# josephg/text-crdt-rust

Measured on AMD Instinct MI355X. Metric: CRDT ops remapped+merged/sec (whole node), higher is better.
Workload: dtype u32

## Files before the change

### text-crdt-rust_amd/csrc/host_plan.h

```cpp
#pragma once
#include <algorithm>
#include <cstring>
#include <string>
#include <unordered_map>
#include <vector>

#include "crdt_types.h"

namespace crdt {

struct WireTxnView {
  u32 agent_name, seq, n_parents, n_ops;
  const u32* parents;
  const u32* ops;
};
struct WireView {
  std::vector<std::string> names;
  std::vector<WireTxnView> txns;
  bool parse(const uint8_t* p, size_t len) {
    size_t off = 0;
    auto rd = [&](u32& v) -> bool {
      if (off + 4 > len) return false;
      std::memcpy(&v, p + off, 4);
      off += 4;
      return true;
    };
    u32 magic, nn;
    if (!rd(magic) || magic != 0x31585452u || !rd(nn)) return false;
    names.resize(nn);
    for (u32 i = 0; i < nn; i++) {
      u32 bl;
      if (!rd(bl) || off + bl > len) return false;
      names[i].assign((const char*)p + off, bl);
      off += (bl + 3) & ~3u;
    }
    u32 nt;
    if (!rd(nt)) return false;
    if (off % 4) return false;
    txns.resize(nt);
    for (u32 t = 0; t < nt; t++) {
      WireTxnView& x = txns[t];
      if (!rd(x.agent_name) || !rd(x.seq) || !rd(x.n_parents) || !rd(x.n_ops)) return false;
      if (x.agent_name >= nn) return false;
      if (off + 8ull * x.n_parents + 24ull * x.n_ops > len) return false;
      x.parents = (const u32*)(p + off);
      off += 8ull * x.n_parents;
      x.ops = (const u32*)(p + off);
      off += 24ull * x.n_ops;
      for (u32 k = 0; k < x.n_parents; k++) if (x.parents[2 * k] >= nn) return false;
      for (u32 k = 0; k < x.n_ops; k++) {
        const u32* o = x.ops + 6 * k;
        if (o[0] > 1 || o[1] >= nn || (o[0] == 0 && o[3] >= nn)) return false;
      }
    }
    return true;
  }
};

struct AgentTable {
  std::vector<std::string> names;
  std::unordered_map<std::string, u32> ids;
  u32 get_or_create(const std::string& n) {
    if (n == "ROOT") return ROOT_AGENT;
    auto it = ids.find(n);
    if (it != ids.end()) return it->second;
    u32 id = (u32)names.size();
    names.push_back(n);
    ids[n] = id;
    return id;
  }
  u32 lookup(const std::string& n) const {
    if (n == "ROOT") return ROOT_AGENT;
    auto it = ids.find(n);
    return it == ids.end() ? UNKNOWN_AGENT : it->second;
  }
  std::vector<u32> ranks() const {
    std::vector<u32> idx(names.size());
    for (u32 i = 0; i < idx.size(); i++) idx[i] = i;
    std::sort(idx.begin(), idx.end(), [&](u32 a, u32 b) { return names[a] < names[b]; });
    std::vector<u32> r(names.size());
    for (u32 i = 0; i < idx.size(); i++) r[idx[i]] = i;
    return r;
  }
};

struct StreamNeeds {
  u64 n_txn = 0, n_ltxn = 0, n_rtxn = 0, n_ops = 0, orders = 0, local_del = 0, remote_del_ops = 0, remote_parents = 0;
  u32 max_ops = 0, max_del = 0, max_len = 0, max_parents = 0;
  u64 probes = 0;
  u64 local_del_ops = 0;
  u32 max_rdel_len = 0;
  std::vector<u32> txns_per_agent;
  void txn_max(u32 ops, u64 del, u64 len, u32 parents) {
    max_ops = std::max(max_ops, ops);
    max_del = (u32)std::min<u64>(std::max<u64>(max_del, del), 0xFFFFFFFFull);
    max_len = (u32)std::min<u64>(std::max<u64>(max_len, len), 0xFFFFFFFFull);
    max_parents = std::max(max_parents, parents);
  }
  void agent_txn(u32 a) {
    if (a >= 0xFFFE) return;
    if (txns_per_agent.size() <= a) txns_per_agent.resize(a + 1, 0);
    txns_per_agent[a]++;
  }
};

inline void encode_lc(std::vector<Rec>& out, StreamNeeds& nd, u32 agent, u32 pos, u32 del, u32 ins) {
  out.push_back(Rec{(REC_LC << 28) | agent, pos, del, ins});
  nd.txn_max(1, del, (u64)del + ins, 0);
  nd.local_del += del;
  nd.local_del_ops += del != 0;
  nd.n_txn++;
  nd.n_ltxn++;
  nd.n_ops++;
  nd.orders += (u64)del + ins;
  nd.agent_txn(agent);
}
inline void encode_local_txn(std::vector<Rec>& out, StreamNeeds& nd, u32 agent, const u32* ops3, u32 nops) {
  u64 span = 0, dels = 0;
  for (u32 k = 0; k < nops; k++) { span += (u64)ops3[3 * k + 1] + ops3[3 * k + 2]; dels += ops3[3 * k + 1]; }
  u32 span32 = span > 0xFFFFFFFFull ? 0xFFFFFFFFu : (u32)span;
  u32 dels32 = dels > 0xFFFFFFFFull ? 0xFFFFFFFFu : (u32)dels;
  if (agent <= 0xFFFFu && span != 0 && span <= 0xFFFFFFFFull &&
      (nops > 1 || (ops3[1] != 0 && ops3[2] != 0))) {
    for (u32 k = 0; k < nops; k++) {
      u32 pos = ops3[3 * k], del = ops3[3 * k + 1], ins = ops3[3 * k + 2];
      if (del) encode_lc(out, nd, agent, pos, del, 0);
      if (ins) encode_lc(out, nd, agent, pos, 0, ins);
    }
    return;
  }
  nd.txn_max(nops, dels, span, 0);
  if (nops == 1 && agent <= 0xFFFFu && span <= 0xFFFFFFFFull) {
    out.push_back(Rec{(REC_LC << 28) | agent, ops3[0], ops3[1], ops3[2]});
    nd.local_del += ops3[1];
    nd.local_del_ops += ops3[1] != 0;
  } else {
    out.push_back(Rec{(REC_LTXN << 28) | (nops & 0x0FFFFFFFu), agent, dels32, span32});
    for (u32 k = 0; k < nops; k++) {
      out.push_back(Rec{REC_LOP << 28, ops3[3 * k], ops3[3 * k + 1], ops3[3 * k + 2]});
      nd.local_del += ops3[3 * k + 1];
      nd.local_del_ops += ops3[3 * k + 1] != 0;
    }
  }
  nd.n_txn++;
  nd.n_ltxn++;
  nd.n_ops += nops;
  nd.orders += span;
  nd.agent_txn(agent);
}

inline void encode_remote(std::vector<Rec>& out, StreamNeeds& nd, AgentTable& at, const WireView& wv) {
  std::vector<u32> cache(wv.names.size(), 0xFFFFFFFFu);
  for (const WireTxnView& t : wv.txns) {
    size_t before = at.names.size();
    u32 author = at.get_or_create(wv.names[t.agent_name]);
    if (at.names.size() != before)
      for (u32 i = 0; i < cache.size(); i++) if (cache[i] == UNKNOWN_AGENT) cache[i] = 0xFFFFFFFFu;
    auto res = [&](u32 ni) -> u32 {
      if (cache[ni] == 0xFFFFFFFFu) cache[ni] = at.lookup(wv.names[ni]);
      return cache[ni];
    };
    u64 tl = 0;
    bool zero = false;
    for (u32 k = 0; k < t.n_ops; k++) {
      u32 len = t.ops[6 * k + 5];
      if (len == 0 || len > 0x0FFFFFFFu) zero = true;
      tl += len;
    }
    u32 tl32 = tl > 0xFFFFFFFFull ? 0xFFFFFFFFu : (u32)tl;
    nd.txn_max(t.n_ops, t.n_ops, tl, t.n_parents);
    u32 has_del = 0;
    for (u32 k = 0; k < t.n_ops; k++)
      if (t.ops[6 * k] != 0) { has_del = 1; nd.max_rdel_len = std::max<u32>(nd.max_rdel_len, tl32); break; }
    if (t.n_ops == 1 && t.n_parents == 1 && author < 0xFFFEu && t.seq >= 1 && res(t.parents[0]) == author &&
        t.parents[1] == t.seq - 1) {
      const u32* o = t.ops;
      u32 len = o[5];
      auto org = [&](u32 ni, u32 seq, u32& enc) -> bool {
        u32 a = res(ni);
        if (a == ROOT_AGENT) { enc = 0xFFFFFFFFu; return true; }
        enc = seq;
        return a == author && seq != 0xFFFFFFFFu;
      };
      u32 e2 = 0, e3 = 0;
      bool ok = len >= 1 && len <= 0x7FFu;
      if (ok && o[0] == 0) ok = org(o[1], o[2], e2) && org(o[3], o[4], e3);
      else if (ok) ok = res(o[1]) == author && o[2] != 0xFFFFFFFFu && (e2 = o[2], true);
      if (ok) {
        out.push_back(Rec{(REC_RC << 28) | ((o[0] ? 1u : 0u) << 27) | (len << 16) | author, t.seq, e2, e3});
        if (o[0]) nd.remote_del_ops++;
        nd.n_txn++;
        nd.n_rtxn++;
        nd.n_ops += 1;
        nd.orders += tl;
        nd.remote_parents += 1;
        nd.agent_txn(author);
        continue;
      }
    }
    if (t.n_ops > RTXN_NOPS_MASK) zero = true;
    out.push_back(Rec{(REC_RTXN << 28) | ((zero ? 1u : 0u) << 27) | (has_del << RTXN_DEL_BIT) | (t.n_ops & RTXN_NOPS_MASK),
                      (author & 0xFFFFu) | ((t.n_parents & 0xFFFFu) << 16), t.seq, tl32});
    for (u32 k = 0; k < t.n_ops; k++) {
      const u32* o = t.ops + 6 * k;
      u32 len = o[5] & 0x0FFFFFFFu;
      if (o[0] == 0) {
        out.push_back(Rec{(REC_RINS << 28) | len, (res(o[1]) & 0xFFFFu) | ((res(o[3]) & 0xFFFFu) << 16), o[2], o[4]});
      } else {
        out.push_back(Rec{(REC_RDEL << 28) | len, res(o[1]) & 0xFFFFu, o[2], 0});
        nd.remote_del_ops++;
      }
    }
    for (u32 k = 0; k < t.n_parents; k++)
      out.push_back(Rec{REC_RPARENT << 28, res(t.parents[2 * k]) & 0xFFFFu, t.parents[2 * k + 1], 0});
    nd.n_txn++;
    nd.n_rtxn++;
    nd.n_ops += t.n_ops;
    nd.orders += tl;
    nd.remote_parents += t.n_parents;
    nd.agent_txn(author);
  }
}

inline void encode_probe(std::vector<Rec>& out, StreamNeeds& nd, u32 pos, u32 agent, u32 seq) {
  out.push_back(Rec{REC_PROBE << 28, pos, agent, seq});
  nd.probes++;
}

inline void encode_gen(std::vector<Rec>& out, StreamNeeds& nd, u32 agent, u32 n_ops, u32 seed) {
  out.push_back(Rec{REC_GEN << 28, agent, n_ops, seed});
  nd.txn_max(1, 10, 10, 0);
  nd.n_txn += n_ops;
  nd.n_ltxn += n_ops;
  nd.n_ops += n_ops;
  nd.orders += 3ull * n_ops;
  nd.local_del += n_ops;
  nd.local_del_ops += n_ops;
  if (agent < 0xFFFE) {
    if (nd.txns_per_agent.size() <= agent) nd.txns_per_agent.resize(agent + 1, 0);
    nd.txns_per_agent[agent] += n_ops;
  }
}

constexpr u32 MAX_LEAVES = 32u * 32u * (ROOT_CAP_MAX - 64u);

struct Caps {
  u32 leaf, blk, map, cwo, arun, del, dd, txn, par, agent, fr;
  u32 ord;
  u32 canon = 0;
};
inline u32 blk_cap_for(u32 leaf_cap) { return leaf_cap / 32 + 2; }
inline u32 root_cap_for(u32 blk_cap) {
  u32 r = (blk_cap + 63u) & ~63u;
  return r < ROOT_CAP_MIN ? ROOT_CAP_MIN : r;
}
inline Caps plan_caps(const StreamNeeds& nd, u32 n_agents, bool track, u32 leaf_div = 48) {
  Caps c;
  u64 leaves = 64 + nd.n_ops / leaf_div;
  c.leaf = (u32)std::min<u64>(leaves, 1 + 2 * nd.n_ops + 1);
  if (c.leaf < 64) c.leaf = 64;
  if (c.leaf > MAX_LEAVES) c.leaf = MAX_LEAVES;
  c.blk = blk_cap_for(c.leaf);
  c.fr = FRONTIER_CAP0;
  c.map = track ? (u32)std::min<u64>(nd.orders + 1, 0xFFFFFFFFull) : 0;
  c.ord = (u32)std::min<u64>(nd.orders + 1, 0xFFFFFFFFull);
  c.cwo = (u32)std::min<u64>(nd.n_txn + 1, 256 + nd.n_txn / 64);
  c.txn = c.cwo;
  u64 arun = 0;
  for (u32 a = 0; a < n_agents; a++) arun += (a < nd.txns_per_agent.size() ? nd.txns_per_agent[a] : 0) + 1;
  c.arun = (u32)arun;
  c.del = (u32)std::min<u64>(std::min<u64>(nd.local_del + nd.remote_del_ops, 2 * (nd.local_del_ops + nd.remote_del_ops) + 64) + 1,
                             0xFFFFFFFFull);
  c.dd = nd.remote_del_ops ? std::max<u32>(4u, (u32)std::min<u64>((2ull * nd.max_rdel_len + 2) / 32 + 3, 0x7FFFFFFFull)) : 0u;
  c.par = (u32)std::min<u64>(nd.remote_parents + nd.n_txn + 64 + 1, 1024 + (nd.remote_parents + nd.n_txn) / 64);
  c.agent = n_agents;
  return c;
}

}
```

### text-crdt-rust_amd/csrc/replay_core.h

```cpp
#pragma once
#include "crdt_types.h"

namespace crdt {

struct Cursor {
  u32 leaf, idx, off;
};
constexpr u32 END_LEAF = 0xFFFFFFFEu;

enum : u32 {
  P_LV = 0, P_DL = 2, P_DV = 4, P_SOL = 6, P_LOF = 8, P_CWO = 10, P_ARUN = 12, P_DELS = 14,
  P_DD = 16, P_TXNS = 18, P_PAR = 20, P_FR = 22, P_AGENTS = 24, P_GROUPS = 26, P_RECS = 28, P_STP = 30,
  P_DDB = 32,
  P_PROBE = P_DDB + 2,
  K_LEAF = P_PROBE + 2, K_MAP, K_CWO, K_TXN, K_DEL, K_DD, K_PAR, K_RECN,
  K_FR,
  P_OAG,
  K_AGMAP = P_OAG + 2,
  P_LAG,
  S_BASE = 64,
  S_STATUS = 64, S_REC_POS, S_N_LEAVES, S_N_BLOCKS, S_NG, S_NEXT_ORDER, S_LEN, S_N_CWO, S_N_DEL,
  S_N_DD, S_N_TXN, S_N_PAR, S_N_FR, S_N_AGENTS, S_N_ITEMS, S_CAP_NEED, S_N_ENTRIES, S_GEN_DONE, S_N_DDB,
  S_PROF0, S_PROF1, S_PROF2, S_PROF3,
  F_FAST,
// ... 1428 lines not shown
    u32 pos0 = g(T_RB_BASE) + b0;
    u32 end = g(T_RB_BASE) + nv;
    while (true) {
      if (pos0 + (nt + 1u) * per <= end) break;
      if (end >= rn) break;
      u32 last = pos0 + (nt - 1u) * per;
      u32 n = rn - last < 64u ? rn - last : 64u;
      u32 t2, l0;
      u32 n2 = w.typing_scan_at(w.at(recs(), last), n, remote, cpt, agent, ow1, o.w3, t2, l0);
      end = last + n;
      if (n2 <= 1u) break;
      total += t2 - l0;
      nt += n2 - 1u;
    }
    return nt;
  }
  CRDT_HD u32 fast_typing(u32 b0, u32 nv, u32 remote, u32 idx, u32 orr, u32 agent, const Rec& o, u32 first) {
    Span e = w.cget(idx);
    if (e.len <= 0) return 0;
    if (e.order + (u32)e.len != first) return 0;
    if (e.orr != orr) return 0;
    u32 total;
    u32 nt = typing_run(b0, nv, remote, agent, o.w1, o, total);
    if (g(K_MAP) - first < total) return 0;
    map_fill(first, total, g(C_LEAF));
    e.len += (i32)total;
    w.cset(idx, e);
    p(C_NOW, g(C_NOW) + total);
    p(C_DIRTY, 1u);
    fast_txn_commit(first, total);
    return nt * per_txn(remote);
  }
  CRDT_HD u32 leaf_delete(u32 idx, u32 off, u32 l) {
    Span e = w.cget(idx);
    u32 n = g(C_N);
    u32 target = e.order + off;
    u32 ha = off > 0u, hc = off + l < (u32)e.len;
    Span pa{e.order, e.ol, e.orr, (i32)off};
    Span dd{target, ha ? target - 1u : e.ol, e.orr, -(i32)l};
    Span pc{target + l, target + l - 1u, e.orr, e.len - (i32)(off + l)};
    Span x0 = ha ? dd : pc;
    u32 m = ha + hc;
    u32 pre = 0;
    Span nx{0, 0, 0, 0};
    if (m != 0u) {
      if (idx + 1u < n) {
        nx = w.cget(idx + 1u);
        Span last = m == 2u ? pc : x0;
        if (can_append_u(last, nx)) {
          nx.order = last.order;
          nx.len += last.len;
          pre = 1;
          m -= 1u;
        }
      }
    }
    if (n + m > (u32)L) return 0;
    w.cset(idx, ha ? pa : dd);
    if (pre) w.cset(idx + 1u, nx);
    if (m) {
      w.cache_shift_right(idx + 1u, n, m);
      p(C_N, n + m);
      w.cset(idx + 1u, x0);
      if (m == 2u) w.cset(idx + 2u, pc);
      inc(S_N_ENTRIES, m);
    }
    p(C_NOW, g(C_NOW) - l);
    p(C_DIRTY, 1u);
    return 1;
  }
  CRDT_HD u32 delete_run_closed(u32 idx, u32 off, u32 t1, u32 k, u32 back) {
    Span E = w.cget(idx);
    u32 n = g(C_N);
    u32 orr = E.orr;
    u32 has_nx = idx + 1u < n;
    Span N0 = w.cget(idx + 1u);
    u32 room = (u32)L - n;
    u32 delta;
    if (back) {
      u32 mid = off + 1u != (u32)E.len ? 1u : 0u;
      u32 p0 = 0u;
      if (mid) {
        if (room == 0u) return 0;
        room -= 1u;
      } else if (has_nx) {
        p0 = can_append_u(Span{t1, t1 - 1u, orr, -1}, N0) ? 1u : 0u;
      }
      u32 kmax = 2u * room + p0;
      k = k < off ? k : off;
      k = k < kmax ? k : kmax;
      if (k < 2u) return 0;
      if (mid) {
        Span pc = truncate(E, off + 1u);
        w.cache_shift_right(idx + 1u, n, 1u);
        w.cset(idx + 1u, pc);
        n += 1u;
        inc(S_N_ENTRIES, 1u);
      }
      delta = p0 ? k / 2u : (k + 1u) / 2u;
      w.cache_shift_right(idx + 1u, n, delta);
      w.cset_lanes(idx + 1u, idx + 1u + delta, [&](u32 lane) {
        u32 q = delta - (lane - idx - 1u);
        u32 jc = p0 ? 2u * q : 2u * q - 1u;
        u32 tc = t1 - (jc - 1u);
        u32 two = jc + 1u <= k ? 1u : 0u;
        return Span{tc - two, tc - 1u, orr, (i32)~two};
      });
      if (p0) w.cset(idx + 1u + delta, Span{t1, N0.ol, N0.orr, N0.len - 1});
      E.len = (i32)(off + 1u - k);
      w.cset(idx, E);
    } else {
      u32 ha = off > 0u;
      if (has_nx && can_append_u(Span{t1 + 1u, t1, orr, E.len - (i32)off - 1}, N0)) return 0;
      u32 kmax = room > ha ? room - ha : 0u;
      k = k < kmax ? k : kmax;
      if (k < 2u) return 0;
      u32 rest = (u32)E.len - off - k;
      u32 cnt = ha + k + (rest != 0u);
      delta = cnt - 1u;
      w.cache_shift_right(idx + 1u, n, delta);
      w.cset_lanes(idx, idx + cnt, [&](u32 lane) {
        u32 p = lane - idx;
        u32 j = p - ha;
        if (ha && p == 0u) return Span{E.order, E.ol, orr, (i32)off};
        if (j < k) return Span{t1 + j, (j == 0u && !ha) ? E.ol : t1 + j - 1u, orr, -1};
        return Span{t1 + k, t1 + k - 1u, orr, (i32)rest};
      });
    }
    p(C_N, n + delta);
    inc(S_N_ENTRIES, delta);
    p(C_NOW, g(C_NOW) - k);
    p(C_DIRTY, 1u);
    return k;
  }
  CRDT_HD u32 fast_deletes(u32 b0, u32 nv, u32 remote, u32 agent, u32 idx, u32 off, u32 l, u32 first, const Rec& o) {
#ifdef CRDT_PROF
    u64 pt0 = w.clock();
#endif
    u32 per = per_txn(remote);
    u32 t1 = w.cget_order(idx) + off;
    u32 split_first = 0;
    if (g(C_N) + 2u > (u32)L) {
      Span e = w.cget(idx);
      u32 n = g(C_N), ha = off > 0u, hc = off + l < (u32)e.len, m = ha + hc;
      if (m && idx + 1u < n) {
        Span last = hc ? Span{t1 + l, t1 + l - 1u, e.orr, e.len - (i32)(off + l)}
                       : Span{t1, ha ? t1 - 1u : e.ol, e.orr, -(i32)l};
        m -= can_append_u(last, w.cget(idx + 1u));
      }
      if (n + m > (u32)L) split_first = 1;
    }
    u32 k = 1, back = 0;
    u32 key = g(T_AGL_KEY);
    u32 delta;
    u32 has_next = b0 + 2u * per <= nv ? 1u : 0u;
    u32 bn = has_next ? b0 + per : b0;
    if (cpt) {
      Rec r2 = w.rec_get(bn);
      delta = remote ? r2.w2 - o.w2 : r2.w1 - o.w1;
    } else {
      Rec o2 = op_at(bn, remote);
      delta = remote ? o2.w2 - o.w2 : o2.w1 - o.w1;
    }
    u32 bk = delta == 0xFFFFFFFFu ? 1u : 0u;
    u32 bad = (l ^ 1u) | (has_next ^ 1u) | ((delta != (remote ? 1u : 0u) ? 1u : 0u) & (bk ^ 1u));
    if (remote) bad |= ((o.w1 & 0xFFFFu) ^ agent) | (o.w2 - key >= g(T_AGL_LEN) ? 1u : 0u);
    if (opq(bad) == 0u) {
      back = opq(bk);
      {
        u32 room = back ? off + 1u : (u32)w.cget_len(idx) - off;
        if (remote) {
          u32 r2 = back ? o.w2 - key + 1u : key + g(T_AGL_LEN) - o.w2;
          room = room < r2 ? room : r2;
        }
        k = w.delete_scan(b0, nv, remote, cpt, agent, delta);
        u32 rn = rec_n();
        u32 pos0 = g(T_RB_BASE) + b0;
        u32 end = g(T_RB_BASE) + nv;
        while (true) {
          if (k >= room) break;
          if (pos0 + (k + 1u) * per <= end) break;
          if (end >= rn) break;
          u32 last = pos0 + (k - 1u) * per;
          u32 n = rn - last < 64u ? rn - last : 64u;
          u32 n2 = w.delete_scan_at(w.at(recs(), last), n, remote, cpt, agent, delta);
          end = last + n;
          if (n2 <= 1u) break;
          k += n2 - 1u;
        }
#ifdef CRDT_PROF

#endif
        k = k < room ? k : room;
      }
    }
#ifdef CRDT_PROF

#endif
    if (g(K_MAP) - first < k * l) return 0;
    if (g(K_DEL) - g(S_N_DEL) < (back ? k : 1u)) return 0;
#ifdef CRDT_PROF
    u64 pt1 = w.clock();
#endif
    u32 done = split_first ? 0u : delete_segment(idx, off, t1, k, back, l);
#ifdef CRDT_PROF
    u64 pt2 = w.clock();
#endif
    CRDT_STAT(9, 1); CRDT_STAT(12, k); CRDT_STAT(13, split_first);
#ifdef CRDT_PROF_LOOP
    u32 lp_gen = 0, lp_split = 0, lp_find = 0, lp_seg = 0;
#endif
    while (done < k) {
#ifdef CRDT_PROF_LOOP
      u64 q0 = w.clock();
#endif
      CRDT_STAT(10, 1);
      if (g(K_LEAF) - g(S_N_LEAVES) < 2u) break;
      Cursor c{g(C_LEAF), idx, off};
      if (done != 0u) {
        if (!find_order(back ? t1 - done : t1 + done, true, c)) break;
      }
      i32 el = w.cget_len(c.idx);
      if (el <= 0) break;
      if (c.off + l > (u32)el) break;
      if (back & (el == 1)) {
        w.cset_len(c.idx, -1);
        p(C_NOW, g(C_NOW) - 1u);
        p(C_DIRTY, 1u);
        done++;
        continue;
      }
      CRDT_STAT(back ? 48 : 49, 1); CRDT_STAT(52, c.off == 0u);
#ifdef CRDT_PROF_LOOP
      u64 q1 = w.clock();
      prof_split = 0;
#endif
      delete_general(c.idx, c.off, l, back);
#ifdef CRDT_PROF_LOOP
      u64 q2 = w.clock();
      lp_gen += (u32)(q2 - q1) - prof_split;
      lp_split += prof_split;
      lp_find += (u32)(q1 - q0);
#endif
      done++;
      if (done == k) break;
      u32 t2 = back ? t1 - done : t1 + done;
      if (back & (c.off != 0u)) c.off -= 1u;
      else if (!find_order(t2, true, c)) break;
      el = w.cget_len(c.idx);
      if (el <= 0) break;
      if (c.off + l > (u32)el) break;
#ifdef CRDT_PROF_LOOP
      u64 q3 = w.clock();
      lp_find += (u32)(q3 - q2);
#endif
      if (back & (c.leaf == g(C_LEAF)) & (l == 1u)) {
        u32 dc = back_cycles(c.idx, t2, k - done);
        CRDT_STAT(57, dc != 0u); CRDT_STAT(58, dc);
        if (dc) {
          done += dc;
          if (done == k) break;
          t2 -= dc;
          c.off -= dc;
        }
      }
      u32 dseg = delete_segment(c.idx, c.off, t2, k - done, back, l);
#ifdef CRDT_PROF_LOOP
      lp_seg += (u32)(w.clock() - q3);
#endif
      CRDT_STAT(53, dseg); CRDT_STAT(54, dseg == 0u);
      done += dseg;
    }
#ifdef CRDT_PROF
    u64 pt3 = w.clock();
#endif
    if (done == 0u) return 0;
    if (back) {
      append_delete(first, t1, 1u);
      if (done > 1u) {
        u32 n = g(S_N_DEL);
        w.st(&w.at(dels(), n - 1u)->len, g(T_DEL_LEN));
        w.st_del_run(w.at(dels(), n), done - 1u, first + 1u, t1 - 1u);
        p(S_N_DEL, n + done - 1u);
        p(T_DEL_KEY, first + done - 1u);
        p(T_DEL_ORDER, t1 - (done - 1u));
        p(T_DEL_LEN, 1u);
      }
    } else {
      append_delete(first, t1, done * l);
    }
    fast_txn_commit(first, done * l);
#ifdef CRDT_PROF
    if (prof_mode == 3u && !prof_gen) {
#ifdef CRDT_PROF_LOOP
      (void)pt0; (void)pt1; (void)pt2; (void)pt3;
      inc(S_PROF0, lp_gen); inc(S_PROF1, lp_split); inc(S_PROF2, lp_find); inc(S_PROF3, lp_seg);
#else
      inc(S_PROF0, (u32)(pt1 - pt0)); inc(S_PROF1, (u32)(pt2 - pt1));
      inc(S_PROF2, (u32)(pt3 - pt2)); inc(S_PROF3, (u32)(w.clock() - pt3));
#endif
    }
#endif
    return done * per;
  }
  CRDT_HD u32 delete_segment(u32 idx, u32 off, u32 t, u32 k, u32 back, u32 l) {
    u32 done = k >= 2u ? delete_run_closed(idx, off, t, k, back) : 0u;
    CRDT_STAT(11, done); CRDT_STAT(14, 1);
    if (done == 0u) {
      for (u32 j = 0; j < k; j++) {
        u32 ij = back ? idx : (j == 0u ? idx : idx + (off > 0u) + j);
        u32 oj = back ? off - j : (j == 0u ? off : 0u);
        u32 tj = back ? t - j : t + j;
        if (w.cget_order(ij) + oj != tj) break;
        if (w.cget_len(ij) <= (i32)oj) break;
        if (!leaf_delete(ij, oj, l)) break;
        done++;
      }
    }
    return done;
  }
  CRDT_HD void delete_general(u32 idx, u32 off, u32 l, u32 back) {
    CRDT_STAT(7, 1);
    Span e = w.cget(idx);
    u32 n = g(C_N);
    u32 t = e.order + off;
    u32 ha = off > 0u ? 1u : 0u, hc = off + l < (u32)e.len ? 1u : 0u;
    Span pa{e.order, e.ol, e.orr, (i32)off};
    Span dd{t, ha ? t - 1u : e.ol, e.orr, -(i32)l};
    Span pc{t + l, t + l - 1u, e.orr, e.len - (i32)(off + l)};
    Span x0 = ha ? dd : pc;
    u32 m = ha + hc;
    u32 pre = 0, pre_vis = 0;
    Span nx{0, 0, 0, 0};
    if (m != 0u) {
      if (idx + 1u < n) {
        nx = w.cget(idx + 1u);
        Span last = m == 2u ? pc : x0;
        if (can_append_u(last, nx)) {
          nx.order = last.order;
          nx.len += last.len;
          pre = 1;
          pre_vis = last.len > 0 ? (u32)last.len : 0u;
          m -= 1u;
        }
      }
    }
    w.cset(idx, ha ? pa : dd);
    if (pre) w.cset(idx + 1u, nx);
    u32 unplaced_vis = (hc && !pre) ? (u32)pc.len : 0u;
    p(C_NOW, g(C_NOW) - l - unplaced_vis);
    p(C_DIRTY, 1u);
// ... 600 lines not shown
```

### text-crdt-rust_amd/csrc/wave_gpu.h

```cpp
#pragma once
#include "crdt_types.h"

namespace crdt {

__device__ __forceinline__ u32 lane_id() { return __lane_id(); }
__device__ __forceinline__ u32 lane_here() {
  u32 l;
  asm volatile("v_mbcnt_lo_u32_b32 %0, -1, 0\n\tv_mbcnt_hi_u32_b32 %0, -1, %0" : "=v"(l));
  return l;
}
__device__ __forceinline__ u32 uni(u32 x) { return __builtin_amdgcn_readfirstlane(x); }
__device__ __forceinline__ u32 rdlane(u32 x, u32 l) { return __builtin_amdgcn_readlane(x, l); }
__device__ int crdt_writelane_i32(int v, int l, int old) __asm("llvm.amdgcn.writelane.i32");
__device__ __forceinline__ u32 wrlane(u32 old, u32 v, u32 l) { return (u32)crdt_writelane_i32((int)v, (int)l, (int)old); }
__device__ __forceinline__ u64 ballot(bool p) { return __builtin_amdgcn_ballot_w64(p); }
__device__ __forceinline__ u32 shfl(u32 v, u32 src) { return __builtin_amdgcn_ds_bpermute((int)(src << 2), (int)v); }

__device__ __forceinline__ u32 wave_umax(u32 v) {
  v = max(v, (u32)__builtin_amdgcn_update_dpp(0u, v, 0x111, 0xf, 0xf, false));
  v = max(v, (u32)__builtin_amdgcn_update_dpp(0u, v, 0x112, 0xf, 0xf, false));
  v = max(v, (u32)__builtin_amdgcn_update_dpp(0u, v, 0x114, 0xf, 0xf, false));
  v = max(v, (u32)__builtin_amdgcn_update_dpp(0u, v, 0x118, 0xf, 0xf, false));
  v = max(v, (u32)__builtin_amdgcn_update_dpp(0u, v, 0x142, 0xa, 0xf, false));
  v = max(v, (u32)__builtin_amdgcn_update_dpp(0u, v, 0x143, 0xc, 0xf, false));
// ... 476 lines not shown
  template <class F> __device__ __forceinline__ void leaf_write_lanes(Span* dst, u32 n, F f) const {
    u32 l = lane();
    Span e = f(l);
    bool in = l < n;
    if (l < (u32)L) *(uint4*)(dst + l) = in ? make_uint4(e.order, e.ol, e.orr, (u32)e.len) : make_uint4(0, 0, 0, 0);
  }
  __device__ __forceinline__ void leaf_prefetch(const Span* p) const {
    typedef __attribute__((address_space(1))) u32 g_u32;
    u32 l = lane();
    if (l < (u32)L) __builtin_amdgcn_global_load_lds((g_u32*)(p + l), pf, 16, 0, 0);
  }
  __device__ __forceinline__ void prefetch_drain() const { asm volatile("s_waitcnt vmcnt(0)" ::: "memory"); }
  __device__ __forceinline__ u32 cache_from_prefetch() {
    asm volatile("s_waitcnt vmcnt(0)" ::: "memory");
    u32 l = lane();
    bool in = l < (u32)L;
    const lds_u32* q = pf + 4u * (l & (u32)(L - 1));
    u32 a = q[0], b = q[1], c = q[2], d = q[3];
    eo = in ? a : 0u; el = in ? b : 0u; er = in ? c : 0u; en = in ? (i32)d : 0;
    return __popcll(ballot(en != 0));
  }
  __device__ __forceinline__ void fill_runs(u32* base, u32 a, u32 b, u32 v) const {
    u32 l = lane();
    u32 ln = l >= a && l < b ? (u32)(en < 0 ? -en : en) : 0u;
    u32 Pi = wave_incl_scan(ln);
    u32 T = rdlane(Pi, 63);
    u32 vb = eo - (Pi - ln);
    for (u32 t = 0; t < T; t += 64) {
      u32 j = t + l;
      u32 m4 = 0;
      for (u32 step = (u32)L / 2u; step; step >>= 1) {
        u32 x = (u32)__builtin_amdgcn_ds_bpermute((int)(m4 + 4u * (step - 1u)), (int)Pi);
        m4 = x <= j ? m4 + 4u * step : m4;
      }
      u32 o = (u32)__builtin_amdgcn_ds_bpermute((int)m4, (int)vb) + j;
      if (j < T) *(u32*)((char*)base + (u64)(o * 4u)) = v;
    }
  }
  __device__ __forceinline__ void cache_clear(u32 a, u32 b) {
    u32 l = lane();
    bool z = l >= a && l < b;
    eo = z ? 0u : eo;
    el = z ? 0u : el;
    er = z ? 0u : er;
    en = z ? 0 : en;
  }
  __device__ __forceinline__ void cache_shift_right(u32 idx, u32 n, u32 k) {
    static_assert(L <= 32, "lane 63 of the cache is always empty");
    u32 l = lane();
    (void)n;
    u32 src = l >= idx + k ? l - k : 63u;
    u32 o = shfl(eo, src), a = shfl(el, src), b = shfl(er, src), c = shfl((u32)en, src);
    bool up = l >= idx;
    eo = up ? o : eo;
    el = up ? a : el;
    er = up ? b : er;
    en = up ? (i32)c : en;
  }

  u32 rx = 0, ry = 0, rz = 0, rw = 0;
  u32 qx = 0, qy = 0, qz = 0, qw = 0;
  __device__ __forceinline__ uint4 rec_lane_load(const Rec* p, u32 n) const {
    u32 l = lane();
    u32 m = n - 1u;
    return *(const uint4*)(p + (l < m ? l : m));
  }
  __device__ __forceinline__ void rec_load2(const Rec* p, u32 n, u32 n_ahead) {
    uint4 v = rec_lane_load(p, n);
    rx = v.x; ry = v.y; rz = v.z; rw = v.w;
    if (n_ahead) {
      uint4 q = rec_lane_load(p + 64, n_ahead);
      qx = q.x; qy = q.y; qz = q.z; qw = q.w;
    }
  }
  __device__ __forceinline__ void rec_slide(u32 d, const Rec* p_ahead, u32 n_ahead) {
    if (d >= 64u) {
      rx = qx; ry = qy; rz = qz; rw = qw;
      d -= 64u;
    }
    if (d) {
      u32 l = lane();
      u32 src = (l + d) & 63u;
      bool own = l + d < 64u;
      u32 ax = shfl(rx, src), ay = shfl(ry, src), az = shfl(rz, src), aw = shfl(rw, src);
      u32 bx = shfl(qx, src), by = shfl(qy, src), bz = shfl(qz, src), bw = shfl(qw, src);
      rx = own ? ax : bx; ry = own ? ay : by; rz = own ? az : bz; rw = own ? aw : bw;
    }
    if (n_ahead) {
      uint4 q = rec_lane_load(p_ahead, n_ahead);
      qx = q.x; qy = q.y; qz = q.z; qw = q.w;
    }
  }
  __device__ __forceinline__ Rec rec_get(u32 k) const {
    return Rec{rdlane(rx, k), rdlane(ry, k), rdlane(rz, k), rdlane(rw, k)};
  }
  __device__ __forceinline__ void balance_tick(u32 remaining) const {
    if constexpr (!HR) balance_board_tick(remaining);
  }
  __device__ __forceinline__ void gen_draws(u32 seed, u32 base) {
    GenDraw d = gen_draw(seed, base + lane());
    rx = d.hi; ry = d.lo; rz = d.r2;
  }
  __device__ __forceinline__ u32 typing_scan_r(u32 X, u32 Y, u32 Z, u32 Q, u32 b0, u32 nv, u32 remote, u32 compact, u32 agent, u32 ow1, u32 ow3,
                                             u32& total) const {
    u32 l = lane();
    if (compact) {
      u32 p0 = shfl(X, l - 1u), p1 = shfl(Y, l - 1u), p3 = shfl(Q, l - 1u);
      bool ok;
      u32 hl;
      if (remote) {
        hl = (X >> 16) & 0x7FFu;
        u32 ra = ow3 == 0xFFFFFFFFu ? 0xFFFFu : agent;
        u32 ubad = (agent | (ra << 16)) != ow1 ? 1u : 0u;
        u32 d = ((X & RC_HDR_MASK) ^ ((REC_RC << 28) | agent)) | (Y ^ (p1 + ((p0 >> 16) & 0x7FFu))) |
                (Z ^ (Y - 1u)) | (Q ^ ow3) | ubad;
        ok = d == 0u && hl != 0u;
      } else {
        hl = Q;
        ok = X == ((REC_LC << 28) | agent) && Z == 0u && Q - 1u < 0xFFFFu && Y == p1 + p3;
      }
      u64 stop = ballot(!ok || l >= nv) & (~1ull << b0);
      u32 f = stop ? (u32)__builtin_ctzll(stop) : 64u;
      total = wave_sum(l - b0 < f - b0 ? hl : 0u);
      return f - b0;
    }
    u32 rel = l - b0;
    u32 per = remote ? 3u : 2u;
    u32 t = remote ? (rel * 43u) >> 7 : rel >> 1;
    u32 r = rel - t * per;
    bool ok;
    if (remote) {
      u32 src = r == 0u ? l - 3u : (r == 1u ? l - 1u : l - 2u);
      u32 hs = shfl(Z, src), hl = shfl(Q, src);
      bool okh = X == ((REC_RTXN << 28) | 1u) && Y == (agent | (1u << 16)) && Z == hs + hl && Q - 1u < 0xFFFFu;
      bool oko = (X >> 28) == REC_RINS && (X & 0x0FFFFFFFu) == hl && Y == ow1 && Q == ow3 && Z == hs - 1u;
      bool okp = X == (REC_RPARENT << 28) && Y == agent && Z == hs - 1u;
      ok = r == 0u ? okh : (r == 1u ? oko : okp);
    } else {
      u32 hl = shfl(Q, l - 1u), ps = shfl(Y, l - 2u), pl = shfl(Q, l - 2u);
      bool okh = X == ((REC_LTXN << 28) | 1u) && Y == agent && Z == 0u && Q - 1u < 0xFFFFu;
      bool oko = X == (REC_LOP << 28) && Z == 0u && Q == hl && Y == ps + pl;
      ok = r == 0u ? okh : oko;
    }
    u64 stop = ballot(l >= b0 + per && (!ok || l >= nv));
    u32 f = stop ? (u32)__builtin_ctzll(stop) : 64u;
    u32 n = remote ? ((f - b0) * 43u) >> 7 : (f - b0) >> 1;
    total = wave_sum(l >= b0 && r == 0u && t < n ? Q : 0u);
    return n;
  }

  __device__ __forceinline__ u32 delete_scan_r(u32 X, u32 Y, u32 Z, u32 Q, u32 b0, u32 nv, u32 remote, u32 compact, u32 agent, u32 delta) const {
    u32 l = lane();
    if (compact) {
      u32 p1 = shfl(Y, l - 1u), p2 = shfl(Z, l - 1u);
      u32 d = remote ? ((X ^ ((REC_RC << 28) | (1u << 27) | (1u << 16) | agent)) | (Y ^ (p1 + 1u)) | (Z ^ (p2 + delta)))
                     : ((X ^ ((REC_LC << 28) | agent)) | (Z ^ 1u) | Q | (Y ^ (p1 + delta)));
      bool ok = d == 0u;
      u64 stop = ballot(!ok || l >= nv) & (~1ull << b0);
      u32 f = stop ? (u32)__builtin_ctzll(stop) : 64u;
      return f - b0;
    }
    u32 rel = l - b0;
    u32 per = remote ? 3u : 2u;
    u32 t = remote ? (rel * 43u) >> 7 : rel >> 1;
    u32 r = rel - t * per;
    bool ok;
    if (remote) {
      u32 ps = shfl(Z, r == 2u ? l - 2u : l - 3u);
      bool okh = X == ((REC_RTXN << 28) | (1u << RTXN_DEL_BIT) | 1u) && Y == (agent | (1u << 16)) && Z == ps + 1u && Q == 1u;
      bool oko = X == ((REC_RDEL << 28) | 1u) && Y == agent && Z == ps + delta;
      bool okp = X == (REC_RPARENT << 28) && Y == agent && Z == ps - 1u;
      ok = r == 0u ? okh : (r == 1u ? oko : okp);
    } else {
      u32 pp = shfl(Y, l - 2u);
      bool okh = X == ((REC_LTXN << 28) | 1u) && Y == agent && Z == 1u && Q == 1u;
      bool oko = X == (REC_LOP << 28) && Z == 1u && Q == 0u && Y == pp + delta;
      ok = r == 0u ? okh : oko;
    }
    u64 stop = ballot(l >= b0 + per && (!ok || l >= nv));
    u32 f = stop ? (u32)__builtin_ctzll(stop) : 64u;
    return remote ? ((f - b0) * 43u) >> 7 : (f - b0) >> 1;
  }
  __device__ __forceinline__ u32 front_scan(u32 b0, u32 nv, u32 agent, u32 len) const {
    u32 l = lane();
    u32 d = (rx ^ ((REC_LC << 28) | agent)) | ry | rz | (rw ^ len);
    u64 stop = ballot(d != 0u || l >= nv) & (~1ull << b0);
    u32 f = stop ? (u32)__builtin_ctzll(stop) : 64u;
    return f - b0;
  }
  __device__ __forceinline__ u32 typing_scan(u32 b0, u32 nv, u32 remote, u32 compact, u32 agent, u32 ow1, u32 ow3,
                                             u32& total) const {
    return typing_scan_r(rx, ry, rz, rw, b0, nv, remote, compact, agent, ow1, ow3, total);
  }
  __device__ __forceinline__ u32 typing_scan_at(const Rec* p, u32 nv, u32 remote, u32 compact, u32 agent, u32 ow1,
                                                u32 ow3, u32& total, u32& len0) const {
    uint4 v = rec_lane_load(p, nv);
    len0 = (compact & remote) ? (rdlane(v.x, 0) >> 16) & 0x7FFu : rdlane(v.w, 0);
    return typing_scan_r(v.x, v.y, v.z, v.w, 0u, nv, remote, compact, agent, ow1, ow3, total);
  }
  __device__ __forceinline__ u32 delete_scan(u32 b0, u32 nv, u32 remote, u32 compact, u32 agent, u32 delta) const {
    return delete_scan_r(rx, ry, rz, rw, b0, nv, remote, compact, agent, delta);
  }
  __device__ __forceinline__ u32 delete_scan_at(const Rec* p, u32 nv, u32 remote, u32 compact, u32 agent, u32 delta) const {
    uint4 v = rec_lane_load(p, nv);
    return delete_scan_r(v.x, v.y, v.z, v.w, 0u, nv, remote, compact, agent, delta);
  }
  __device__ __forceinline__ static u32 wave_shr1(u32 v) {
    u32 r = (u32)__builtin_amdgcn_update_dpp(0, (int)v, 0x138, 0xf, 0xf, false);
    asm("" : "+v"(r));
    return r;
  }
  __device__ __forceinline__ void decode_window(u32 nv, u32 s_typ) {
    u32 l = lane();
    u32 p0 = wave_shr1(rx), p1 = wave_shr1(ry), p3 = wave_shr1(rw);
    u32 dt = ((rx & RC_HDR_MASK) ^ ((REC_RC << 28) | (p0 & 0xFFFFu))) | (ry ^ (p1 + ((p0 >> 16) & 0x7FFu))) |
             (rz ^ (ry - 1u)) | (rw ^ p3);
    bool in = l - 1u < nv - 1u;
    u64 mt = ballot(in & (dt == 0u) & ((rx & (0x7FFu << 16)) != 0u));
    xs(s_typ, (u32)mt); xs(s_typ + 1u, (u32)(mt >> 32));
  }
  __device__ __forceinline__ u64 win_mask(u32 s) const { return ((u64)rdlane(x2, s - 127u) << 32) | rdlane(x2, s - 128u); }
  __device__ __forceinline__ static u32 mask_run(u64 m, u32 b0) {
    u64 stop = ~m & (~1ull << b0);
    return (stop ? (u32)__builtin_ctzll(stop) : 64u) - b0;
  }
  __device__ __forceinline__ u32 typing_scan_m(u32 b0, u32 s_typ, u32& total) const {
    u32 n = mask_run(win_mask(s_typ), b0);
    u32 e = b0 + n - 1u;
    total = rdlane(ry, e) + ((rdlane(rx, e) >> 16) & 0x7FFu) - rdlane(ry, b0);
    return n;
  }

  __device__ __forceinline__ u32 frontier_advance(u32* f, u32 nfr, u32 f0, const u32* pp, u32 np, u32 p0, u32 first,
                                                  u32 last, u32 cap, u32& nf0) const {
    u32 l = lane();
    bool in = l < nfr;
    u32 fv = f[in ? l : 0u];
    fv = l == 0u ? f0 : fv;
    if (ballot(in && fv == first)) return 0u;
    u32 pv = np > 1u ? pp[l < np ? l : 0u] : 0u;
    pv = l == 0u ? p0 : pv;
    bool hit = false;
    for (u32 j = 0; j < np; j++) hit |= fv == rdlane(pv, j);
    u64 keep = ballot(in && !hit);
    u32 m = (u32)__popcll(keep);
    if (m + 1u > cap) return INVALID;
    nf0 = m ? rdlane(fv, (u32)__builtin_ctzll(keep)) : last;
    u32 at = (u32)__popcll(keep & ((1ull << l) - 1ull));
    if (((keep >> l) & 1ull) && at >= 1u) f[at] = fv;
    if (m) f[m] = last;
    return m + 1u;
  }
  static constexpr u32 FR_L0 = FR_S0 - 64u;
  __device__ __forceinline__ void fr_lanes_load(const u32* f, u32 n) {
    u32 l = lane();
    bool mine = (l >= FR_L0) & (l < FR_L0 + n - 1u);
    u32 v = f[mine ? l - FR_L0 + 1u : 0u];
    x1 = mine ? v : x1;
  }
  __device__ __forceinline__ void fr_lanes_store(u32* f, u32 n) const {
    u32 l = lane();
    if ((l >= FR_L0) & (l < FR_L0 + n - 1u)) f[l - FR_L0 + 1u] = x1;
  }
  __device__ __forceinline__ u32 frontier_advance_x(u32 nfr, u32 f0, const u32* pp, u32 np, u32 p0, u32 first,
                                                    u32 last, u32 cap, u32& nf0, u32* f) {
    u32 l = lane();
    bool in = l < nfr;
    u32 fv = shfl(x1, l + FR_L0 - 1u);
    fv = l == 0u ? f0 : fv;
    if (ballot(in && fv == first)) return 0u;
    u32 pv = np > 1u ? pp[l < np ? l : 0u] : 0u;
    pv = l == 0u ? p0 : pv;
    bool hit = false;
    for (u32 j = 0; j < np; j++) hit |= fv == rdlane(pv, j);
    u64 keep = ballot(in && !hit);
    u32 m = (u32)__popcll(keep);
    if (m + 1u > cap) return INVALID;
    nf0 = m ? rdlane(fv, (u32)__builtin_ctzll(keep)) : last;
    u32 at = (u32)__popcll(keep & ((1ull << l) - 1ull));
    bool mv = ((keep >> l) & 1ull) && at >= 1u;
    if (m <= FR_LANES) {
      u32 moved = (u32)__builtin_amdgcn_ds_permute((int)((mv ? FR_L0 + at - 1u : 0u) << 2), (int)fv);
      if (m) x1 = ((l >= FR_L0) & (l < FR_L0 + m - 1u)) ? moved : l == FR_L0 + m - 1u ? last : x1;
    } else {
      if (mv) f[at] = fv;
      f[m] = last;
    }
    return m + 1u;
  }
  __device__ __forceinline__ void st_del_run(DelRun* p, u32 cnt, u32 key0, u32 t0) const {
    for (u32 j = lane(); j < cnt; j += 64) {
      u32* q = (u32*)(p + j);
      q[0] = key0 + j;
      q[1] = t0 - j;
      q[2] = 1u;
    }
  }

  __device__ __forceinline__ lds_u32* rblk() const { return rt; }
  __device__ __forceinline__ lds_u32* rcnt() const { return rt + rcap; }
  __device__ __forceinline__ lds_u32* rvis() const { return rt + 2 * rcap; }
  __device__ __forceinline__ lds_u32* gob() const { return rt + 3 * rcap; }
  __device__ __forceinline__ lds_u32* trow() const { return rt; }
  __device__ __forceinline__ lds_u32* tcnt() const { return rt + rcap; }
  __device__ __forceinline__ lds_u32* tvis() const { return rt + 2 * rcap; }
  __device__ __forceinline__ u32 ntop() const { return uni(rt[3 * rcap]); }
  __device__ __forceinline__ void set_ntop(u32 v) const { rt[3 * rcap] = v; }
  __device__ __forceinline__ u32 nrows() const { return uni(rt[3 * rcap + 1]); }
  __device__ __forceinline__ void set_nrows(u32 v) const { rt[3 * rcap + 1] = v; }
// ... 408 lines not shown
```

Measured before the change: 34.09 billion.

## Precompute remote compact delete run lengths on host into record hints

During host encoding, a backward pass over remote compact records stores in the spare word the length and direction of each run of consecutive single-char deletes. The device delete path for remote compact records then reads that run length directly instead of doing wave-wide scans and repeated rescans across 64-record windows. The compact scan helper is reduced to the local case. The cost is an extra host pass over the records and reliance on the otherwise unused w3 field of compact remote records.

```diff
diff --git a/text-crdt-rust_amd/csrc/host_plan.h b/text-crdt-rust_amd/csrc/host_plan.h
--- a/text-crdt-rust_amd/csrc/host_plan.h
+++ b/text-crdt-rust_amd/csrc/host_plan.h
@@ -149,7 +149,29 @@
   nd.agent_txn(agent);
 }
 
+inline void hint_delete_runs(std::vector<Rec>& out, size_t from) {
+  const u32 DEL1 = (REC_RC << 28) | (1u << 27) | (1u << 16);
+  u32 mn = 0, dn = 0;
+  for (size_t j = out.size(); j-- > from;) {
+    Rec& r = out[j];
+    if ((r.w0 >> 27) != ((REC_RC << 1) | 1u)) { mn = 0; continue; }
+    u32 m = 1, d = 0;
+    if (mn && (r.w0 & ~0xFFFFu) == DEL1 && out[j + 1].w0 == r.w0 && out[j + 1].w1 == r.w1 + 1u) {
+      u32 step = out[j + 1].w2 - r.w2;
+      if (step == 1u || step == 0xFFFFFFFFu) {
+        d = step;
+        m = (mn >= 2u && dn == step) ? mn + 1u : 2u;
+        if (m > 0x7FFFFFFFu) m = 0x7FFFFFFFu;
+      }
+    }
+    r.w3 = ((d == 0xFFFFFFFFu ? 1u : 0u) << 31) | m;
+    mn = m;
+    dn = d;
+  }
+}
+
 inline void encode_remote(std::vector<Rec>& out, StreamNeeds& nd, AgentTable& at, const WireView& wv) {
+  const size_t from = out.size();
   std::vector<u32> cache(wv.names.size(), 0xFFFFFFFFu);
   for (const WireTxnView& t : wv.txns) {
     size_t before = at.names.size();
@@ -220,6 +242,7 @@
     nd.remote_parents += t.n_parents;
     nd.agent_txn(author);
   }
+  hint_delete_runs(out, from);
 }
 
 inline void encode_probe(std::vector<Rec>& out, StreamNeeds& nd, u32 pos, u32 agent, u32 seq) {
diff --git a/text-crdt-rust_amd/csrc/replay_core.h b/text-crdt-rust_amd/csrc/replay_core.h
--- a/text-crdt-rust_amd/csrc/replay_core.h
+++ b/text-crdt-rust_amd/csrc/replay_core.h
@@ -1604,51 +1604,57 @@
     }
     u32 k = 1, back = 0;
     u32 key = g(T_AGL_KEY);
-    u32 delta;
-    u32 has_next = b0 + 2u * per <= nv ? 1u : 0u;
-    u32 bn = has_next ? b0 + per : b0;
-    if (cpt) {
-      Rec r2 = w.rec_get(bn);
-      delta = remote ? r2.w2 - o.w2 : r2.w1 - o.w1;
+    if (remote && cpt) {
+      u32 m = o.w3 & 0x7FFFFFFFu;
+      u32 bad = (l ^ 1u) | (m < 2u ? 1u : 0u) | (o.w2 - key >= g(T_AGL_LEN) ? 1u : 0u);
+      if (opq(bad) == 0u) {
+        back = o.w3 >> 31;
+        u32 room = back ? off + 1u : (u32)w.cget_len(idx) - off;
+        u32 r2 = back ? o.w2 - key + 1u : key + g(T_AGL_LEN) - o.w2;
+        room = room < r2 ? room : r2;
+        k = m < room ? m : room;
+      }
     } else {
-      Rec o2 = op_at(bn, remote);
-      delta = remote ? o2.w2 - o.w2 : o2.w1 - o.w1;
-    }
-    u32 bk = delta == 0xFFFFFFFFu ? 1u : 0u;
-    u32 bad = (l ^ 1u) | (has_next ^ 1u) | ((delta != (remote ? 1u : 0u) ? 1u : 0u) & (bk ^ 1u));
-    if (remote) bad |= ((o.w1 & 0xFFFFu) ^ agent) | (o.w2 - key >= g(T_AGL_LEN) ? 1u : 0u);
-    if (opq(bad) == 0u) {
-      back = opq(bk);
-      {
-        u32 room = back ? off + 1u : (u32)w.cget_len(idx) - off;
-        if (remote) {
-          u32 r2 = back ? o.w2 - key + 1u : key + g(T_AGL_LEN) - o.w2;
-          room = room < r2 ? room : r2;
+      u32 delta;
+      u32 has_next = b0 + 2u * per <= nv ? 1u : 0u;
+      u32 bn = has_next ? b0 + per : b0;
+      if (cpt) {
+        Rec r2 = w.rec_get(bn);
+        delta = r2.w1 - o.w1;
+      } else {
+        Rec o2 = op_at(bn, remote);
+        delta = remote ? o2.w2 - o.w2 : o2.w1 - o.w1;
+      }
+      u32 bk = delta == 0xFFFFFFFFu ? 1u : 0u;
+      u32 bad = (l ^ 1u) | (has_next ^ 1u) | ((delta != (remote ? 1u : 0u) ? 1u : 0u) & (bk ^ 1u));
+      if (remote) bad |= ((o.w1 & 0xFFFFu) ^ agent) | (o.w2 - key >= g(T_AGL_LEN) ? 1u : 0u);
+      if (opq(bad) == 0u) {
+        back = opq(bk);
+        {
+          u32 room = back ? off + 1u : (u32)w.cget_len(idx) - off;
+          if (remote) {
+            u32 r2 = back ? o.w2 - key + 1u : key + g(T_AGL_LEN) - o.w2;
+            room = room < r2 ? room : r2;
+          }
+          k = w.delete_scan(b0, nv, remote, cpt, agent, delta);
+          u32 rn = rec_n();
+          u32 pos0 = g(T_RB_BASE) + b0;
+          u32 end = g(T_RB_BASE) + nv;
+          while (true) {
+            if (k >= room) break;
+            if (pos0 + (k + 1u) * per <= end) break;
+            if (end >= rn) break;
+            u32 last = pos0 + (k - 1u) * per;
+            u32 n = rn - last < 64u ? rn - last : 64u;
+            u32 n2 = w.delete_scan_at(w.at(recs(), last), n, remote, cpt, agent, delta);
+            end = last + n;
+            if (n2 <= 1u) break;
+            k += n2 - 1u;
+          }
+          k = k < room ? k : room;
         }
-        k = w.delete_scan(b0, nv, remote, cpt, agent, delta);
-        u32 rn = rec_n();
-        u32 pos0 = g(T_RB_BASE) + b0;
-        u32 end = g(T_RB_BASE) + nv;
-        while (true) {
-          if (k >= room) break;
-          if (pos0 + (k + 1u) * per <= end) break;
-          if (end >= rn) break;
-          u32 last = pos0 + (k - 1u) * per;
-          u32 n = rn - last < 64u ? rn - last : 64u;
-          u32 n2 = w.delete_scan_at(w.at(recs(), last), n, remote, cpt, agent, delta);
-          end = last + n;
-          if (n2 <= 1u) break;
-          k += n2 - 1u;
-        }
-#ifdef CRDT_PROF
-
-#endif
-        k = k < room ? k : room;
-      }
-    }
-#ifdef CRDT_PROF
-
-#endif
+      }
+    }
     if (g(K_MAP) - first < k * l) return 0;
     if (g(K_DEL) - g(S_N_DEL) < (back ? k : 1u)) return 0;
 #ifdef CRDT_PROF
diff --git a/text-crdt-rust_amd/csrc/wave_gpu.h b/text-crdt-rust_amd/csrc/wave_gpu.h
--- a/text-crdt-rust_amd/csrc/wave_gpu.h
+++ b/text-crdt-rust_amd/csrc/wave_gpu.h
@@ -652,9 +652,8 @@
   __device__ __forceinline__ u32 delete_scan_r(u32 X, u32 Y, u32 Z, u32 Q, u32 b0, u32 nv, u32 remote, u32 compact, u32 agent, u32 delta) const {
     u32 l = lane();
     if (compact) {
-      u32 p1 = shfl(Y, l - 1u), p2 = shfl(Z, l - 1u);
-      u32 d = remote ? ((X ^ ((REC_RC << 28) | (1u << 27) | (1u << 16) | agent)) | (Y ^ (p1 + 1u)) | (Z ^ (p2 + delta)))
-                     : ((X ^ ((REC_LC << 28) | agent)) | (Z ^ 1u) | Q | (Y ^ (p1 + delta)));
+      u32 p1 = shfl(Y, l - 1u);
+      u32 d = (X ^ ((REC_LC << 28) | agent)) | (Z ^ 1u) | Q | (Y ^ (p1 + delta));
       bool ok = d == 0u;
       u64 stop = ballot(!ok || l >= nv) & (~1ull << b0);
       u32 f = stop ? (u32)__builtin_ctzll(stop) : 64u;
```

After: 35.83 billion, median of 6. 1.05x the previous value.
